# theo2021/OnDA

Hardware: AMD Instinct MI355X
Metric: adaptation-step images/sec (fwd+bwd+proto) 512x1024 bs=4 (higher is better)
Workload: dtype f32 (f16x2 split emulation); 1 GPU; hybrid_switch adaptation step (step + update_ema), 1024x512, bs=4 per micro-batch, 1 micro-batch(es) per GPU and optimizer step, dynamic branch, DeepLabV2-ResNet50 ProDA head, random-init weights; global_batch=4, parallelism=dp1, branch=dynamic, micro_batches_per_gpu=1, inputs=resident in HBM

## Files before the change

include/onda_hip.h:

```cpp
#ifndef ONDA_HIP_H
#define ONDA_HIP_H

#include <stdint.h>

#ifdef __cplusplus
extern "C" {
#endif

typedef void* onda_stream_t;

#define ONDA_OK 0
#define ONDA_EINVAL (-1)
#define ONDA_EALIGN (-2)

typedef struct OndaConv {
  int B, Hi, Wi, Cin;
  int Ho, Wo, Cout;
  int kh, kw, stride, dil, pad;
  int ldx;
  int ldy;
  int ldr;
  int out_os;
  int Hf, Wf;
  int relu;
// ... 83 lines not shown
int onda_conv2d_wgrad(const float* x, const float* dy, float* slabs, int lddy, int splitk,
                      const OndaConv* c, onda_stream_t s);
int onda_wgrad_reduce(const float* slabs, float* dw, int splitk, int Cout, int taps, int Cin,
                      int Cout_real, int Cin_real, int flat_k, int accumulate, onda_stream_t s);

int onda_pack_weight_fwd(const float* w_oihw, float* dst, int Cout, int Cin, int taps, int Cout_pad, int Kp,
                         onda_stream_t s);
int onda_pack_weight_dgrad(const float* w_oihw, float* dst, int Cout, int Cin, int taps, int Cout_pad,
                           onda_stream_t s);

int onda_stem_im2col(const float* x_nchw, float* col, int B, int H, int W, int Ho, int Wo, int Kp, onda_stream_t s);

int onda_bn_finalize(const float* partials, int tiles, int C, int64_t count, float eps, float* mean, float* invstd,
                     float* running_mean, float* running_var, int64_t* num_batches_tracked, float momentum,
                     onda_stream_t s);
int onda_bn_stats(const float* x, int64_t M, int C, int ldx, float* partials, int* tiles_out, onda_stream_t s);
int onda_bn_apply(const float* x, const float* mean, const float* invstd, const float* gamma, const float* beta,
                  const float* residual, float* out, int64_t M, int C, int relu, float* amax, onda_stream_t s);
int onda_bn_fold(const float* gamma, const float* beta, const float* running_mean, const float* running_var,
                 float eps, float* scale, float* shift, int C, onda_stream_t s);
int64_t onda_bn_bwd_ws(int64_t M, int C);
int onda_bn_bwd(const float* dout, const float* out, const float* x, const float* mean, const float* invstd,
                const float* gamma, float* dx, float* dres, float* ws, int64_t M, int C, int relu, float* amax, onda_stream_t s);

int64_t onda_gn_ws(int B, int64_t HW, int C);
int onda_gn_fwd(const float* x, int ldx, const float* gamma, const float* beta, const float* chmul, float* out, int ldo,
                float* mean, float* rstd, float* ws, int B, int64_t HW, int C, int groups, float eps, int relu,
                float* amax ,
                onda_stream_t s);
int onda_gn_bwd(const float* dout, int lddo, const float* out, int ldo, const float* x, int ldx, const float* gamma,
                const float* chmul, const float* mean, const float* rstd, float* dx, float* dgamma, float* dbeta,
                float* ws, int B, int64_t HW, int C, int groups, int relu, onda_stream_t s);

int onda_maxpool_fwd(const float* x, float* y, uint8_t* idx, int B, int Hi, int Wi, int C, int Ho, int Wo,
                     onda_stream_t s);
int onda_maxpool_fwd_limbs(const float* x, const float* xamax, void* yl, uint8_t* idx, int B, int Hi, int Wi, int C, int Ho, int Wo,
                           onda_stream_t s);
int onda_maxpool_bwd(const float* dy, const uint8_t* idx, float* dx, int B, int Hi, int Wi, int C, int Ho, int Wo,
                     onda_stream_t s);

int64_t onda_colsum_ws(int B, int64_t HW, int C);
int onda_colsum(const float* x, int ldx, const float* y, int ldy, float* out, float alpha, float* ws, int B,
                int64_t HW, int C, onda_stream_t s);
int onda_se_fc_fwd(const float* pooled, const float* w1, const float* b1, const float* w2, const float* b2,
                   float* hidden, float* gate, int B, int C, int R, onda_stream_t s);
int onda_se_fc_bwd(const float* dgate, const float* pooled, const float* hidden, const float* gate, const float* w1,
                   const float* w2, float* dw1, float* db1, float* dw2, float* db2, float* dpooled, float* ws,
                   float dpooled_scale, int B, int C, int R, onda_stream_t s);
int onda_chan_scale(const float* x, const float* gate, const float* add, float* out, int B, int64_t HW, int C,
                    onda_stream_t s);
int onda_chan_scale_limbs(const float* x, const float* gate, void* out, int64_t out_plane, const float* x_amax, int B, int64_t HW,
                          int C, onda_stream_t s);

int onda_upsample_fwd(const float* logits, int ldl, float* out_nchw, int B, int h, int w, int K, int H, int W,
                      onda_stream_t s);
int onda_upsample_bwd(const float* dout_nchw, float* dlogits, int ldl, int B, int h, int w, int K, int H, int W,
                      onda_stream_t s);
int onda_upsample_ce_fused(int w, int W);
int64_t onda_upsample_ce_ws(int B, int H, int W);
int onda_upsample_ce_fwd(const float* logits, int ldl, const uint8_t* labels, float* result, float* ws, int B, int h, int w, int K,
                         int H, int W, onda_stream_t s);
int64_t onda_upsample_ce_bwd_ws(int B, int w, int K, int H);
int onda_upsample_ce_bwd(const float* logits, int ldl, const uint8_t* labels, const float* result, const float* gscale, float w_ce,
                         float* dlogits, float* ws, int B, int h, int w, int K, int H, int W, onda_stream_t s);
int onda_upsample_argmax(const float* logits, int ldl, uint8_t* cls, int B, int h, int w, int K, int H, int W,
                         onda_stream_t s);
// ... 75 lines not shown
```

onda_amd/_lib.py:

```python
import ctypes
import os
from ctypes import POINTER, Structure, c_char_p, c_float, c_int, c_int64, c_void_p

HERE = os.path.dirname(os.path.abspath(__file__))
LIB_PATH = os.environ.get("ONDA_LIB_PATH") or os.path.join(HERE, "libonda_hip.so")

P = c_void_p
I, L, F = c_int, c_int64, c_float


class OndaConv(Structure):
    _fields_ = [(n, c_int) for n in ("B Hi Wi Cin Ho Wo Cout kh kw stride dil pad ldx ldy ldr out_os Hf Wf relu").split()] + \
               [("run_if", c_void_p), ("stat_split", c_int64), ("plain_schedule", c_int), ("pix_table", c_void_p),
                ("pix_stride", c_int64)]


class OndaSwitchCfg(Structure):
    _fields_ = [("limit", c_int), ("level_kind", c_int), ("use_exp", c_int), ("pad_", c_int), ("exp_const", ctypes.c_double),
                ("one_minus_exp_const", ctypes.c_double), ("taps_total", ctypes.c_double), ("gray_lo", ctypes.c_double),
                ("gray_hi", ctypes.c_double), ("dev_threshold", ctypes.c_double)]


class OndaLimbOut(Structure):
    _fields_ = [("out", c_void_p), ("out_plane", c_int64), ("out_bound", c_void_p), ("out_amax", c_void_p), ("kb", c_void_p),
# ... 32 lines not shown
    "onda_switch_step": (I, [P, P, P, I, P, POINTER(OndaSwitchCfg), P, P]),
    "onda_select_prior": (I, [P, P, F, P, F, P, L, P]),
    "onda_gate_scalar": (I, [P, P, P, P]),
    "onda_conv_l2_variant": (I, [L, I]),
    "onda_conv_l2_kernel_id": (I, [L, I, I, I]),
    "onda_conv_l2_tiles_m": (I, [L, I, I, I]),
    "onda_conv_l2_tiles_m_split": (I, [L, I, I, I, L, I, POINTER(c_int)]),
    "onda_conv_l2_live_fraction": (ctypes.c_double, [POINTER(OndaConv), I]),
    "onda_conv_wgrad_l2_live_fraction": (ctypes.c_double, [POINTER(OndaConv), I]),
    "onda_conv_wgrad_l2_variant": (I, [I, I]),
    "onda_conv2d_wgrad_l2_table_stride": (L, [POINTER(OndaConv)]),
    "onda_conv2d_wgrad_l2_table": (I, [POINTER(OndaConv), P, P]),
    "onda_conv2d_wgrad_l2": (I, [P, L, P, P, L, P, P, I, I, POINTER(OndaConv), P]),
    "onda_conv2d_fwd_l2": (I, [P, L, P, P, P, P, P, P, P, P, I, P, P, POINTER(OndaConv), P]),
    "onda_bn_finalize_l2": (I, [P, I, I, L, F, P, P, P, P, P, F, P, P, P, I, P, P, L, I, I, P, I, P]),
    "onda_bn_apply_l2": (I, [P, P, P, P, P, P, L, P, P, L, P, L, I, I, P, L, P]),
    "onda_bn_bwd_l2_ws": (L, [L, I]),
    "onda_bn_train_l2": (I, [P, P, I, F, P, P, P, P, P, F, P, P, P, P, I, P, P, P, L, I, P, L, I, I, P]),
    "onda_bn_bwd_l2": (I, [P, P, L, P, P, P, P, P, P, L, P, P, P, L, I, I, P, L, I, P]),
    "onda_conv2d_wgrad": (I, [P, P, P, I, I, POINTER(OndaConv), P]),
    "onda_wgrad_reduce": (I, [P, P, I, I, I, I, I, I, I, I, P]),
    "onda_pack_weight_fwd": (I, [P, P, I, I, I, I, I, P]),
    "onda_pack_weight_dgrad": (I, [P, P, I, I, I, I, P]),
    "onda_stem_im2col": (I, [P, P, I, I, I, I, I, I, P]),
    "onda_bn_finalize": (I, [P, I, I, L, F, P, P, P, P, P, F, P]),
    "onda_bn_stats": (I, [P, L, I, I, P, POINTER(c_int), P]),
    "onda_bn_apply": (I, [P, P, P, P, P, P, P, L, I, I, P, P]),
    "onda_bn_fold": (I, [P, P, P, P, F, P, P, I, P]),
    "onda_bn_bwd_ws": (L, [L, I]),
    "onda_bn_bwd": (I, [P, P, P, P, P, P, P, P, P, L, I, I, P, P]),
    "onda_gn_ws": (L, [I, L, I]),
    "onda_gn_fwd": (I, [P, I, P, P, P, P, I, P, P, P, I, L, I, I, F, I, P, P]),
    "onda_gn_bwd": (I, [P, I, P, I, P, I, P, P, P, P, P, P, P, P, I, L, I, I, I, P]),
    "onda_maxpool_fwd": (I, [P, P, P, I, I, I, I, I, I, P]),
    "onda_maxpool_fwd_limbs": (I, [P, P, P, P, I, I, I, I, I, I, P]),
    "onda_maxpool_bwd": (I, [P, P, P, I, I, I, I, I, I, P]),
    "onda_colsum_ws": (L, [I, L, I]),
    "onda_colsum": (I, [P, I, P, I, P, F, P, I, L, I, P]),
    "onda_se_fc_fwd": (I, [P, P, P, P, P, P, P, I, I, I, P]),
    "onda_se_fc_bwd": (I, [P, P, P, P, P, P, P, P, P, P, P, P, F, I, I, I, P]),
    "onda_chan_scale": (I, [P, P, P, P, I, L, I, P]),
    "onda_chan_scale_limbs": (I, [P, P, P, L, P, I, L, I, P]),
    "onda_upsample_fwd": (I, [P, I, P, I, I, I, I, I, I, P]),
    "onda_upsample_bwd": (I, [P, P, I, I, I, I, I, I, I, P]),
    "onda_upsample_argmax": (I, [P, I, P, I, I, I, I, I, I, P]),
    "onda_upsample_ce_fused": (I, [I, I]),
    "onda_upsample_ce_ws": (L, [I, I, I]),
    "onda_upsample_ce_fwd": (I, [P, I, P, P, P, I, I, I, I, I, I, P]),
    "onda_upsample_ce_bwd_ws": (L, [I, I, I, I]),
    "onda_upsample_ce_bwd": (I, [P, I, P, P, P, F, P, P, I, I, I, I, I, I, P]),
    "onda_upsample_argmax_hist": (I, [P, I, P, P, P, I, I, I, I, I, I, P]),
    "onda_softmax_stats": (I, [P, I, P, I, P, P, P, L, I, P]),
    "onda_seg_loss_fwd": (I, [P, I, P, P, P, L, I, P]),
    "onda_seg_loss_bwd": (I, [P, I, P, P, P, F, F, F, P, L, I, P]),
    "onda_target_loss_fwd": (I, [P, I, P, I, F, F, F, F, P, P, L, I, P]),
    "onda_target_loss_bwd": (I, [P, I, P, I, F, F, F, F, P, P, P, L, I, P]),
    "onda_proto_sigma": (I, [P, P, P, P, I, I, P]),
    "onda_proto_assign_blocks": (I, [L]),
    "onda_proto_assign": (I, [P, I, P, I, P, P, I, F, F, P, P, P, P, L, I, I, P]),
    "onda_proto_distances": (I, [P, I, P, P, I, P, L, I, I, P]),
    "onda_proto_sums_ws": (L, [L, I, I]),
    "onda_proto_class_sums": (I, [P, I, P, P, P, P, L, I, I, P]),
    "onda_proto_ema": (I, [P, P, P, P, F, I, I, P]),
    "onda_proto_append": (I, [P, P, P, P, P, I, I, P]),
    "onda_sgd_multi": (I, [P, I, F, F, F, L, P]),
    "onda_ema_multi": (I, [P, I, L, P]),
# ... 46 lines not shown
```

onda_amd/csrc/norm.hip:

```cpp
#include "common.h"

namespace {

struct ColPlan {
  int cx, ry, gridx, chunks;
  int64_t rows_per_chunk;
};

static inline ColPlan col_plan(int B, int64_t HW, int C) {
  ColPlan p;
  const int c4 = C / 4;
  p.cx = 1;
  while (p.cx < c4 && p.cx < 64) p.cx <<= 1;
  p.ry = 256 / p.cx;
  p.gridx = (c4 + p.cx - 1) / p.cx;
  int64_t target = 2048 / ((int64_t)B * p.gridx);
  if (target < 1) target = 1;
  int64_t rpc = (HW + target - 1) / target;
  const int64_t min_rows = (int64_t)p.ry * 8;
  if (rpc < min_rows) rpc = min_rows;
  p.rows_per_chunk = rpc;
  p.chunks = (int)((HW + rpc - 1) / rpc);
  return p;
}
// ... 241 lines not shown
  if (threadIdx.x != 0) return;
  s1 = ((red[0][0] + red[0][1]) + red[0][2]) + red[0][3];
  s2 = ((red[1][0] + red[1][1]) + red[1][2]) + red[1][3];
  const double mu = s1 / count;
  double var = s2 / count - mu * mu;
  if (var < 0.0) var = 0.0;
  mean[idx] = (float)mu;
  rstd[idx] = (float)(1.0 / sqrt(var + (double)eps));
}

__global__ __launch_bounds__(256) void gn_apply_kernel(const float* __restrict__ x, int ldx,
                                                       const float* __restrict__ gamma, const float* __restrict__ beta,
                                                       const float* __restrict__ chmul, float* __restrict__ out,
                                                       int ldo, const float* __restrict__ mean,
                                                       const float* __restrict__ rstd, int64_t HW, int C, int groups,
                                                       size_t total4, int relu, float* __restrict__ amax) {
  const int c4 = C / 4, cpg = C / groups;
  float mx = 0.f;
  for (size_t e = (size_t)blockIdx.x * blockDim.x + threadIdx.x; e < total4; e += (size_t)gridDim.x * blockDim.x) {
    const int col = (int)(e % c4) * 4;
    const size_t row = e / c4;
    const int b = (int)(row / HW);
    const int gi = b * groups + col / cpg;
    f32x4 v = (LD4(x + row * ldx + col) - mean[gi]) * rstd[gi] * LD4(gamma + col) + LD4(beta + col);
    if (relu) {
#pragma unroll
      for (int j = 0; j < 4; ++j) v[j] = fmaxf(v[j], 0.f);
    }
    if (chmul) v *= LD4(chmul + (size_t)b * C + col);
    *reinterpret_cast<f32x4*>(out + row * ldo + col) = v;
    mx = fmaxf(fmaxf(mx, fmaxf(fabsf(v[0]), fabsf(v[1]))), fmaxf(fabsf(v[2]), fabsf(v[3])));
  }
  if (amax != nullptr) amax_update(amax, mx);
}

__global__ __launch_bounds__(256) void pair_finalize_kernel(const float* __restrict__ partials, int chunks, int B,
                                                            int C, float* __restrict__ AB) {
  const int lane = threadIdx.x & 63;
  const int i = blockIdx.x * 4 + (threadIdx.x >> 6);
  if (i >= B * C) return;
  const int b = i / C, ch = i % C;
  double s1 = 0.0, s2 = 0.0;
  for (int k = lane; k < chunks; k += 64) {
    const size_t base = (((size_t)b * chunks + k) * 2) * C + ch;
    s1 += (double)partials[base];
    s2 += (double)partials[base + C];
  }
  s1 = wave_sum_d(s1);
  s2 = wave_sum_d(s2);
  if (lane == 0) {
    AB[((size_t)b * 2 + 0) * C + ch] = (float)s1;
    AB[((size_t)b * 2 + 1) * C + ch] = (float)s2;
  }
}

__global__ void gn_bwd_group_kernel(const float* __restrict__ AB, int B, int C, int groups,
                                    const float* __restrict__ gamma, float* __restrict__ dgamma,
                                    float* __restrict__ dbeta, float* __restrict__ gsum ) {
  for (int ch = threadIdx.x; ch < C; ch += blockDim.x) {
    float da = 0.f, db = 0.f;
    for (int b = 0; b < B; ++b) {
      db += AB[((size_t)b * 2 + 0) * C + ch];
      da += AB[((size_t)b * 2 + 1) * C + ch];
    }
    if (dgamma) dgamma[ch] = da;
    if (dbeta) dbeta[ch] = db;
// ... 12 lines not shown
  }
}

__global__ __launch_bounds__(256) void gn_bwd_apply_kernel(const float* __restrict__ dout, int lddo,
                                                           const float* __restrict__ out, int ldo,
                                                           const float* __restrict__ x, int ldx,
                                                           const float* __restrict__ gamma,
                                                           const float* __restrict__ chmul,
                                                           const float* __restrict__ mean,
                                                           const float* __restrict__ rstd,
                                                           const float* __restrict__ gsum, float* __restrict__ dx,
                                                           int64_t HW, int C, int groups, size_t total4, float inv_n,
                                                           int relu) {
  const int c4 = C / 4, cpg = C / groups;
  for (size_t e = (size_t)blockIdx.x * blockDim.x + threadIdx.x; e < total4; e += (size_t)gridDim.x * blockDim.x) {
    const int col = (int)(e % c4) * 4;
    const size_t row = e / c4;
    const int b = (int)(row / HW);
    const int gi = b * groups + col / cpg;
    f32x4 g = LD4(dout + row * lddo + col);
    if (relu) {
      const f32x4 ov = LD4(out + row * ldo + col);
#pragma unroll
      for (int j = 0; j < 4; ++j) g[j] = ov[j] > 0.f ? g[j] : 0.f;
    }
    if (chmul) g *= LD4(chmul + (size_t)b * C + col);
    const float rs = rstd[gi];
    const f32x4 xh = (LD4(x + row * ldx + col) - mean[gi]) * rs;
    const f32x4 v = rs * (LD4(gamma + col) * g - (gsum[gi * 2] + xh * gsum[gi * 2 + 1]) * inv_n);
    *reinterpret_cast<f32x4*>(dx + row * C + col) = v;
  }
}

__global__ __launch_bounds__(256) void colsum_finalize_kernel(const float* __restrict__ partials, int chunks, int B,
                                                              int C, float alpha, float* out) {
  const int lane = threadIdx.x & 63;
  const int i = blockIdx.x * 4 + (threadIdx.x >> 6);
  if (i >= B * C) return;
  const int b = i / C, ch = i % C;
  double s = 0.0;
  for (int k = lane; k < chunks; k += 64) s += (double)partials[(((size_t)b * chunks + k) * 2) * C + ch];
  s = wave_sum_d(s);
  if (lane == 0) out[i] = (float)(s * (double)alpha);
}

static inline unsigned ew_grid(size_t total4) {
  size_t g = (total4 + 255) / 256;
  if (g > 8192) g = 8192;
  if (g < 1) g = 1;
  return (unsigned)g;
}

}

extern "C" {

int onda_bn_finalize(const float* partials, int tiles, int C, int64_t count, float eps, float* mean, float* invstd,
                     float* running_mean, float* running_var, int64_t* nbt, float momentum, onda_stream_t s) {
  ONDA_REQUIRE(partials && mean && invstd && tiles >= 1 && C >= 1 && count >= 1);
  hipLaunchKernelGGL(bn_finalize_kernel, dim3((C + 3) / 4), dim3(256), 0, ONDA_STREAM(s), partials, tiles, C,
                     (double)count, eps, mean, invstd, running_mean, running_var, nbt, momentum);
  return ONDA_LAUNCH_RESULT();
}

int onda_bn_stats(const float* x, int64_t M, int C, int ldx, float* partials, int* tiles_out, onda_stream_t s) {
  ONDA_REQUIRE(x && partials && tiles_out && C % 4 == 0 && ldx % 4 == 0);
// ... 54 lines not shown
  const ColPlan p = col_plan(B, HW, C);
  SqStats f{x, HW, ldx};
  int rc = launch_colreduce(f, B, HW, C, ws, p, ONDA_STREAM(s));
  if (rc) return rc;
  hipLaunchKernelGGL(gn_finalize_kernel, dim3(B * groups), dim3(256), 0, ONDA_STREAM(s), ws, p.chunks, B,
                     C, groups, (double)HW * (C / groups), eps, mean, rstd);
  const size_t total4 = (size_t)B * HW * C / 4;
  hipLaunchKernelGGL(gn_apply_kernel, dim3(ew_grid(total4)), dim3(256), 0, ONDA_STREAM(s), x, ldx, gamma, beta, chmul,
                     out, ldo, mean, rstd, HW, C, groups, total4, relu, amax);
  return ONDA_LAUNCH_RESULT();
}

int onda_gn_bwd(const float* dout, int lddo, const float* out, int ldo, const float* x, int ldx, const float* gamma,
                const float* chmul, const float* mean, const float* rstd, float* dx, float* dgamma, float* dbeta,
                float* ws, int B, int64_t HW, int C, int groups, int relu, onda_stream_t s) {
  ONDA_REQUIRE(dout && x && gamma && mean && rstd && dx && ws && (!relu || out));
  ONDA_REQUIRE(C % groups == 0 && (C / groups) % 4 == 0 && ldx % 4 == 0 && lddo % 4 == 0);
  const ColPlan p = col_plan(B, HW, C);
  float* AB = ws + (size_t)B * p.chunks * 2 * C;
  float* gsum = AB + (size_t)B * 2 * C;
  GnBwdRed f{dout, out, x, chmul, mean, rstd, HW, lddo, ldo, ldx, C, groups, relu};
  int rc = launch_colreduce(f, B, HW, C, ws, p, ONDA_STREAM(s));
  if (rc) return rc;
  hipLaunchKernelGGL(pair_finalize_kernel, dim3((B * C + 3) / 4), dim3(256), 0, ONDA_STREAM(s), ws, p.chunks, B, C, AB);
  hipLaunchKernelGGL(gn_bwd_group_kernel, dim3(1), dim3(256), 0, ONDA_STREAM(s), AB, B, C, groups, gamma, dgamma, dbeta,
                     gsum);
  const size_t total4 = (size_t)B * HW * C / 4;
  hipLaunchKernelGGL(gn_bwd_apply_kernel, dim3(ew_grid(total4)), dim3(256), 0, ONDA_STREAM(s), dout, lddo, out, ldo, x,
                     ldx, gamma, chmul, mean, rstd, gsum, dx, HW, C, groups, total4,
                     (float)(1.0 / ((double)HW * (C / groups))), relu);
  return ONDA_LAUNCH_RESULT();
}

int64_t onda_colsum_ws(int B, int64_t HW, int C) {
  const ColPlan p = col_plan(B, HW, C);
  return (int64_t)B * p.chunks * 2 * C;
}

int onda_colsum(const float* x, int ldx, const float* y, int ldy, float* out, float alpha, float* ws, int B,
                int64_t HW, int C, onda_stream_t s) {
  ONDA_REQUIRE(x && out && ws && C % 4 == 0 && ldx % 4 == 0 && (!y || ldy % 4 == 0));
  const ColPlan p = col_plan(B, HW, C);
  ProdSum f{x, y, HW, ldx, ldy};
  int rc = launch_colreduce(f, B, HW, C, ws, p, ONDA_STREAM(s));
  if (rc) return rc;
  hipLaunchKernelGGL(colsum_finalize_kernel, dim3((B * C + 3) / 4), dim3(256), 0, ONDA_STREAM(s), ws, p.chunks, B, C,
                     alpha, out);
  return ONDA_LAUNCH_RESULT();
}

}
```

onda_amd/ops/conv.py:

```python
import ctypes
import os
from ctypes import byref

import torch

from .. import _lib
from .._lib import OndaConv, OndaLimbOut, call, query
from . import _state
from ._state import BN_EPS, GN_EPS, GN_GROUPS, HEAD_PAD, STEM_K
from .core import _conv_ws, _desc, _group_split, _l2_name, _launch, _p, _require_cuda, _stream, as_nhwc, conv_out_size, nhwc_ld
from .limbs import H2Weight, Limbs, amax_slot, is_limb_only, known_amax, limb_only, limbs_of, tag_amax
from .tables import _table


def _use_l2(wp, cin):
    return isinstance(wp, H2Weight) and _state.H2_PATH == "dma" and cin % 32 == 0


def _pack_h2(weight, rows_pad, kp, dgrad, cout_pad):
    cout, cin, kh, kw = weight.shape
    w = weight.detach().contiguous()
    slot = known_amax(weight)
    if slot is None:
        slot = amax_slot(weight.device, long_lived=True)
# ... 264 lines not shown
            "onda_conv2d_wgrad", _p(x), _p(dy), _p(slabs), nhwc_ld(dy), sk, byref(d), _stream(),
            tag=("wgrad", M, Co, Cin, k, stride, dil, sk))


def _wgrad_finish(slabs, into, sk, Co, taps, Cin, cout_real, cin_real, flat_k, k, device):
    if into is not None:
        call("onda_wgrad_reduce", _p(slabs), _p(into), sk, Co, taps, Cin, cout_real, cin_real, flat_k, 1, _stream())
        return None
    if flat_k:
        dw = torch.empty(cout_real, cin_real, 7, 7, device=device, dtype=torch.float32)
    else:
        dw = torch.empty(cout_real, cin_real, k, k, device=device, dtype=torch.float32)
    call("onda_wgrad_reduce", _p(slabs), _p(dw), sk, Co, taps, Cin, cout_real, cin_real, flat_k, 0, _stream())
    return dw


def _accumulate_target(weight):
    g = weight.grad
    if g is not None and g.is_contiguous() and g.dtype == torch.float32 and g.shape == weight.shape:
        return g
    return None


def colsum(x, y=None, alpha=1.0, per_image=False):
    B, H, W, C = x.shape
    nb, hw = (B, H * W) if per_image else (1, B * H * W)
    ws = torch.empty(query("onda_colsum_ws", nb, hw, C), device=x.device, dtype=torch.float32)
    out = torch.empty(nb, C, device=x.device, dtype=torch.float32)
    call("onda_colsum", _p(x), nhwc_ld(x), _p(y), nhwc_ld(y) if y is not None else 0, _p(out), float(alpha), _p(ws),
         nb, hw, C, _stream())
    return out if per_image else out[0]


class _PackCache:

    def __init__(self):
        self.key_f = self.key_d = None
        self.fwd = self.dgrad = None

    @staticmethod
    def _key(w):
        return (w.data_ptr(), w._version, w.device, _state.CONV_MODE)

    def get_fwd(self, w, cout_pad=None, kp=None):
        k = self._key(w)
        if self.key_f != k:
            self.fwd, self.key_f = pack_weight_fwd(w, cout_pad, kp), k
        return self.fwd

    def get_dgrad(self, w, cout_pad=None):
        k = self._key(w)
        if self.key_d != k:
            self.dgrad, self.key_d = pack_weight_dgrad(w, cout_pad), k
        return self.dgrad

    def __deepcopy__(self, memo):
        return _PackCache()


class ModelPacker:

    def __init__(self, convs):
        self.convs = [c for c in convs if c.weight.shape[0] % 32 == 0 and c.weight.shape[1] % 32 == 0]
        self.bufs = {}

    def refresh(self, need_dgrad):
# ... 33 lines not shown
            self._keep.append(w)
        table = _table(ents, _lib.OndaPackEntry, dev)
        call("onda_pack_weights_h2_multi", _p(table), len(ents), biggest, _stream())
        self._keep = []


class Conv2dFn(torch.autograd.Function):

    @staticmethod
    def forward(ctx, x, weight, bias, cache, stride, dil, pad, want_stats, cout_pad):
        cout, cin, k, _ = weight.shape
        co = cout_pad or cout
        wp = cache.get_fwd(weight, cout_pad)
        y, stats, _tiles = conv_forward(x, wp, k, stride, dil, pad, co, shift=_pad_vec(bias, co), want_stats=want_stats)
        ctx.save_for_backward(x, weight)
        ctx.xscale = known_amax(x)
        hit = getattr(x, "_onda_limbs", None)
        ctx.xlimbs = hit[1] if hit is not None and hit[0] == x._version else None
        ctx.weight_param = weight
        ctx.sink = _sink_of(x) if ctx.needs_input_grad[0] else None
        ctx.cache, ctx.geom, ctx.has_bias = cache, (k, stride, dil, pad, cout, cin, cout_pad), bias is not None
        ctx.set_materialize_grads(False)
        if want_stats:
            ctx.mark_non_differentiable(stats)
            return y, stats
        return y, None

    @staticmethod
    def backward(ctx, dy, _dstats):
        if dy is None:
            return (None,) * 9
        x, weight = ctx.saved_tensors
        k, stride, dil, pad, cout, cin, cout_pad = ctx.geom
        if not is_limb_only(dy):
            dy = as_nhwc(dy)
        dx = dw = db = None
        if ctx.needs_input_grad[0]:
            sink = ctx.sink
            wpd = ctx.cache.get_dgrad(weight, cout_pad)
            if sink is not None and sink.buf is not None:
                conv_dgrad(dy, wpd, k, stride, dil, pad, cin, x.shape[1:3], accumulate=sink.buf)
                _sink_done(sink)
            else:
                dx = _sink_give(sink, conv_dgrad(dy, wpd, k, stride, dil, pad, cin, x.shape[1:3]), True)
        if ctx.needs_input_grad[1]:
            into = _accumulate_target(ctx.weight_param)
            dw = conv_wgrad(x, dy, k, stride, dil, pad, cout, cin, into=into, xscale=ctx.xscale, xlimbs=ctx.xlimbs)
            if into is not None and _state.GRAD_READY is not None:
                _state.GRAD_READY(ctx.weight_param)
        if ctx.has_bias and ctx.needs_input_grad[2]:
            db = colsum(dy)[:cout]
        return dx, dw, db, None, None, None, None, None, None


def _pad_vec(v, n):
    if v is None or v.numel() == n:
        return v
    out = torch.zeros(n, device=v.device, dtype=v.dtype)
    out[: v.numel()] = v.detach()
    return out


def stem_patches(x_nchw, Ho, Wo, l2):
    hit = getattr(x_nchw, "_onda_patches", None)
    key = (x_nchw._version, bool(l2), Ho, Wo)
    if hit is not None and hit[0] == key:
        return hit[1]
    B, _, H, W = x_nchw.shape
    dev = x_nchw.device
    if l2:
        amax = amax_slot(dev)
        call("onda_absmax", _p(x_nchw), 1, x_nchw.numel(), x_nchw.numel(), _p(amax), _stream())
        M = B * Ho * Wo
        planes = torch.empty(2, M, STEM_K, device=dev, dtype=torch.float16)
        call("onda_stem_im2col_l2", _p(x_nchw), _p(amax), _p(planes), M * STEM_K, B, H, W, Ho, Wo, STEM_K, _stream())
        col = limb_only((B, Ho, Wo, STEM_K), dev, Limbs(planes, amax, STEM_K, M * STEM_K))
    else:
        col = torch.empty(B, Ho, Wo, STEM_K, device=dev, dtype=torch.float32)
        call("onda_stem_im2col", _p(x_nchw), _p(col), B, H, W, Ho, Wo, STEM_K, _stream())
    try:
        x_nchw._onda_patches = (key, col)
    except AttributeError:
        pass
    return col
# ... 53 lines not shown
```

onda_amd/ops/limbs.py:

```python
import ctypes
import os
from ctypes import byref

import torch

from .. import _lib
from .._lib import OndaConv, OndaLimbOut, call, query
from . import _state
from ._state import BN_EPS, GN_EPS, GN_GROUPS, HEAD_PAD, STEM_K
from .core import _p, _stream, nhwc_ld


class H2Weight:
    __slots__ = ("limbs", "amax")

    def __init__(self, limbs, amax):
        self.limbs, self.amax = limbs, amax


_AMAX_POOL = {}


AMAX_SLOTS = 2048
AMAX_POOL_TENSORS = 16384
# ... 12 lines not shown


def amax_slot(device, long_lived=False):
    key = (str(device), bool(long_lived))
    pool = _AMAX_POOL.get(key)
    if pool is None or pool[1] + AMAX_SLOTS > pool[0].numel():
        pool = _AMAX_POOL[key] = _new_amax_pool(device, WEIGHT_POOL_TENSORS if long_lived else AMAX_POOL_TENSORS)
    if pool[2] is not None:
        cur = torch.cuda.current_stream()
        if cur.cuda_stream not in pool[3]:
            cur.wait_event(pool[2])
            pool[3].add(cur.cuda_stream)
    i = pool[1]
    pool[1] = i + AMAX_SLOTS
    return pool[0][i:i + AMAX_SLOTS]


def reserve_amax_slots(device, n):
    pool = _AMAX_POOL.get((str(device), False))
    if pool is None or pool[1] + n * AMAX_SLOTS > pool[0].numel():
        _AMAX_POOL[(str(device), False)] = _new_amax_pool(device)


def tag_amax(t, slot):
    try:
        t._onda_scale = (t._version, slot)
    except AttributeError:
        pass
    return t


def known_amax(t):
    hit = getattr(t, "_onda_scale", None)
    return hit[1] if hit is not None and hit[0] == t._version else None


def activation_scale(x):
    slot = known_amax(x)
    if slot is not None:
        return slot
    B, H, W, C = x.shape
    slot = amax_slot(x.device)
    call("onda_absmax", _p(x), B * H * W, C, nhwc_ld(x), _p(slot), _stream())
    tag_amax(x, slot)
    return slot


class Limbs:
    __slots__ = ("planes", "amax", "ld", "plane", "true_amax")

    def __init__(self, planes, amax, ld, plane, true_amax=None):
        self.planes, self.amax, self.ld, self.plane = planes, amax, ld, plane
        self.true_amax = true_amax if true_amax is not None else amax


def activation_limbs(x):
    hit = getattr(x, "_onda_limbs", None)
    if hit is not None and hit[0] == x._version:
        return hit[1]
    amax = activation_scale(x)
    B, H, W, C = x.shape
    rows = B * H * W
    planes = torch.empty(2, rows, C, device=x.device, dtype=torch.float16)
    call("onda_split_h2", _p(x), rows, C, nhwc_ld(x), _p(planes), C, rows * C, _p(amax), _stream())
    lb = Limbs(planes, amax, C, rows * C)
    try:
# ... 52 lines not shown
```

onda_amd/ops/norm.py:

```python
import ctypes
import os
from ctypes import byref

import torch

from .. import _lib
from .._lib import OndaConv, OndaLimbOut, call, query
from . import _state
from ._state import BN_EPS, GN_EPS, GN_GROUPS, HEAD_PAD, STEM_K
from .core import _group_split, _p, _stream, as_nhwc, nhwc_ld
from .limbs import Limbs, _stat_tile_rows, amax_slot, is_limb_only, known_amax, limb_mode, limb_only, limbs_of, tag_amax
from .conv import _sink_give, _sink_of, colsum


class BNTrainFn(torch.autograd.Function):

    @staticmethod
    def _groups(B, H, W):
        split, M = _group_split(B, H, W), B * H * W
        return [(0, M)] if not split else [(0, split), (split, M - split)]

    @staticmethod
    def forward(ctx, y, stats, gamma, beta, residual, relu, running, momentum):
        B, H, W, C = y.shape
        groups = BNTrainFn._groups(B, H, W)
        G = len(groups)
        mean = torch.empty(G, C, device=y.device, dtype=torch.float32)
        invstd = torch.empty_like(mean)
        out = torch.empty_like(y)
        res = as_nhwc(residual) if residual is not None else None
        if res is not None and nhwc_ld(res) != C:
            res = res.contiguous()
        if G > 1 and (nhwc_ld(y) != C or not y.is_contiguous()):
            raise RuntimeError("onda_amd: row groups need a dense conv output")
        amax = amax_slot(y.device) if _state.CONV_MODE == "f16x2" else None
        for g, (r0, rows) in enumerate(groups):
            part, nrows = stats, stats.shape[0]
            if G > 1:
                bm = _stat_tile_rows(stats)
                if groups[1][0] % bm == 0 and stats.shape[1] == 2:
                    ts = groups[1][0] // bm
                    part = stats[:ts] if g == 0 else stats[ts:]
                    nrows = part.shape[0]
                else:
                    part = torch.empty(query("onda_bn_bwd_ws", rows, C), device=y.device, dtype=torch.float32)
# ... 144 lines not shown
        ctx.save_for_backward(idx)
        ctx.in_shape = (B, Hi, Wi, C)
        if limbs and slot is not None and limb_mode(C):
            planes = torch.empty(2, B * Ho * Wo, C, device=x.device, dtype=torch.float16)
            call("onda_maxpool_fwd_limbs", _p(x), _p(slot), _p(planes), _p(idx), B, Hi, Wi, C, Ho, Wo, _stream())
            return limb_only((B, Ho, Wo, C), x.device, Limbs(planes, slot, C, B * Ho * Wo * C))
        y = torch.empty(B, Ho, Wo, C, device=x.device, dtype=torch.float32)
        call("onda_maxpool_fwd", _p(x), _p(y), _p(idx), B, Hi, Wi, C, Ho, Wo, _stream())
        if slot is not None:
            tag_amax(y, slot)
        return y

    @staticmethod
    def backward(ctx, dy):
        (idx,) = ctx.saved_tensors
        B, Hi, Wi, C = ctx.in_shape
        dy = dy.contiguous()
        dx = torch.empty(B, Hi, Wi, C, device=dy.device, dtype=torch.float32)
        call("onda_maxpool_bwd", _p(dy), _p(idx), _p(dx), B, Hi, Wi, C, dy.shape[1], dy.shape[2], _stream())
        return dx, None


class GNConcatFn(torch.autograd.Function):

    @staticmethod
    def forward(ctx, relu, chmul, *args):
        n = len(args) // 3
        ys, gammas, betas = args[:n], args[n:2 * n], args[2 * n:]
        B, H, W, C = ys[0].shape
        HW = H * W
        cat = torch.empty(B, H, W, C * n, device=ys[0].device, dtype=torch.float32)
        ws = torch.empty(query("onda_gn_ws", B, HW, C), device=cat.device, dtype=torch.float32)
        amax = amax_slot(cat.device) if _state.CONV_MODE == "f16x2" else None
        means, rstds = [], []
        for i in range(n):
            mean = torch.empty(B * GN_GROUPS, device=cat.device, dtype=torch.float32)
            rstd = torch.empty_like(mean)
            sl = cat[..., i * C:(i + 1) * C]
            call("onda_gn_fwd", _p(ys[i]), nhwc_ld(ys[i]), _p(gammas[i]), _p(betas[i]), _p(chmul), _p(sl), C * n,
                 _p(mean), _p(rstd), _p(ws), B, HW, C, GN_GROUPS, GN_EPS, int(relu), _p(amax), _stream())
            means.append(mean)
            rstds.append(rstd)
        if amax is not None:
            tag_amax(cat, amax)
        ctx.save_for_backward(cat, chmul, *ys, *gammas, *means, *rstds)
        ctx.n, ctx.relu = n, relu
        return cat

    @staticmethod
    def backward(ctx, dcat):
        n = ctx.n
        saved = ctx.saved_tensors
        cat, chmul = saved[0], saved[1]
        ys, gammas = saved[2:2 + n], saved[2 + n:2 + 2 * n]
        means, rstds = saved[2 + 2 * n:2 + 3 * n], saved[2 + 3 * n:2 + 4 * n]
        B, H, W, C = ys[0].shape
        HW = H * W
        dcat = as_nhwc(dcat)
        ldd = nhwc_ld(dcat)
        ws = torch.empty(query("onda_gn_ws", B, HW, C), device=cat.device, dtype=torch.float32)
        dys, dgs, dbs = [], [], []
        for i in range(n):
            dx = torch.empty(B, H, W, C, device=cat.device, dtype=torch.float32)
            dg = torch.empty(C, device=cat.device, dtype=torch.float32)
            db = torch.empty_like(dg)
            call("onda_gn_bwd", dcat.data_ptr() + 4 * i * C, ldd, cat.data_ptr() + 4 * i * C, C * n, _p(ys[i]),
                 nhwc_ld(ys[i]), _p(gammas[i]), _p(chmul), _p(means[i]), _p(rstds[i]), _p(dx), _p(dg), _p(db), _p(ws),
                 B, HW, C, GN_GROUPS, int(ctx.relu), _stream())
            dys.append(dx)
            dgs.append(dg)
            dbs.append(db)
        return (None, None, *dys, *dgs, *dbs)




class SEScaleFn(torch.autograd.Function):

    @staticmethod
    def forward(ctx, x, w1, b1, w2, b2):
        B, H, W, C = x.shape
        R = w1.shape[0]
        pooled = colsum(x, alpha=1.0 / (H * W), per_image=True)
        hidden = torch.empty(B, R, device=x.device, dtype=torch.float32)
        gate = torch.empty(B, C, device=x.device, dtype=torch.float32)
        call("onda_se_fc_fwd", _p(pooled), _p(w1), _p(b1), _p(w2), _p(b2), _p(hidden), _p(gate), B, C, R, _stream())
        slot = known_amax(x)
        if slot is not None and limb_mode(C) and x.is_contiguous():
            planes = torch.empty(2, B * H * W, C, device=x.device, dtype=torch.float16)
            call("onda_chan_scale_limbs", _p(x), _p(gate), _p(planes), B * H * W * C, _p(slot), B, H * W, C, _stream())
            out = limb_only((B, H, W, C), x.device, Limbs(planes, slot, C, B * H * W * C))
        else:
            out = torch.empty_like(x)
            call("onda_chan_scale", _p(x), _p(gate), None, _p(out), B, H * W, C, _stream())
        ctx.save_for_backward(x, pooled, hidden, gate, w1, w2)
        return out

    @staticmethod
    def backward(ctx, dout):
        x, pooled, hidden, gate, w1, w2 = ctx.saved_tensors
        B, H, W, C = x.shape
        R = w1.shape[0]
        dout = dout.contiguous()
        dgate = colsum(dout, x, per_image=True)
        dw1, db1 = torch.empty_like(w1), torch.empty(R, device=x.device, dtype=torch.float32)
        dw2, db2 = torch.empty_like(w2), torch.empty(C, device=x.device, dtype=torch.float32)
        dpooled = torch.empty(B, C, device=x.device, dtype=torch.float32)
        ws = torch.empty(B * R, device=x.device, dtype=torch.float32)
        call("onda_se_fc_bwd", _p(dgate), _p(pooled), _p(hidden), _p(gate), _p(w1), _p(w2), _p(dw1), _p(db1), _p(dw2),
             _p(db2), _p(dpooled), _p(ws), 1.0 / (H * W), B, C, R, _stream())
        dx = torch.empty_like(x)
        call("onda_chan_scale", _p(dout), _p(gate), _p(dpooled), _p(dx), B, H * W, C, _stream())
        return dx, dw1, db1, dw2, db2
```

Baseline: 42.43 images/s.

## Fuse per-channel column sums and amax into GroupNorm apply kernels

The GroupNorm forward and backward apply kernels now also write per-chunk column partial sums, and in backward an amax. Those partials are tagged on the output tensors and reused later. The SE pooling reads them instead of re-reading the concatenated activation, and the conv bias gradient uses the column sums of the GN backward dx instead of launching a separate colsum pass. This removes extra full-tensor read passes over large activations, at the cost of block reductions and partial-buffer writes inside the apply kernels.

```diff
diff --git a/include/onda_hip.h b/include/onda_hip.h
--- a/include/onda_hip.h
+++ b/include/onda_hip.h
@@ -139,6 +139,16 @@
                 const float* chmul, const float* mean, const float* rstd, float* dx, float* dgamma, float* dbeta,
                 float* ws, int B, int64_t HW, int C, int groups, int relu, onda_stream_t s);
 
+int onda_gn_colsum_chunks(int B, int64_t HW, int C);
+int onda_gn_fwd_colsum(const float* x, int ldx, const float* gamma, const float* beta, const float* chmul, float* out, int ldo,
+                       float* mean, float* rstd, float* ws, int B, int64_t HW, int C, int groups, float eps, int relu,
+                       float* amax, float* colpart, int ldp, onda_stream_t s);
+int onda_gn_bwd_colsum(const float* dout, int lddo, const float* out, int ldo, const float* x, int ldx, const float* gamma,
+                       const float* chmul, const float* mean, const float* rstd, float* dx, float* dgamma, float* dbeta,
+                       float* ws, int B, int64_t HW, int C, int groups, int relu, float* amax, float* colpart, int ldp,
+                       onda_stream_t s);
+int onda_colpart_finalize(const float* colpart, int chunks, int ldp, int B, int C, float alpha, float* out, onda_stream_t s);
+
 int onda_maxpool_fwd(const float* x, float* y, uint8_t* idx, int B, int Hi, int Wi, int C, int Ho, int Wo,
                      onda_stream_t s);
 int onda_maxpool_fwd_limbs(const float* x, const float* xamax, void* yl, uint8_t* idx, int B, int Hi, int Wi, int C, int Ho, int Wo,
diff --git a/onda_amd/_lib.py b/onda_amd/_lib.py
--- a/onda_amd/_lib.py
+++ b/onda_amd/_lib.py
@@ -88,6 +88,10 @@
     "onda_gn_ws": (L, [I, L, I]),
     "onda_gn_fwd": (I, [P, I, P, P, P, P, I, P, P, P, I, L, I, I, F, I, P, P]),
     "onda_gn_bwd": (I, [P, I, P, I, P, I, P, P, P, P, P, P, P, P, I, L, I, I, I, P]),
+    "onda_gn_colsum_chunks": (I, [I, L, I]),
+    "onda_gn_fwd_colsum": (I, [P, I, P, P, P, P, I, P, P, P, I, L, I, I, F, I, P, P, I, P]),
+    "onda_gn_bwd_colsum": (I, [P, I, P, I, P, I, P, P, P, P, P, P, P, P, I, L, I, I, I, P, P, I, P]),
+    "onda_colpart_finalize": (I, [P, I, I, I, I, F, P, P]),
     "onda_maxpool_fwd": (I, [P, P, P, I, I, I, I, I, I, P]),
     "onda_maxpool_fwd_limbs": (I, [P, P, P, P, I, I, I, I, I, I, P]),
     "onda_maxpool_bwd": (I, [P, P, P, I, I, I, I, I, I, P]),
diff --git a/onda_amd/csrc/norm.hip b/onda_amd/csrc/norm.hip
--- a/onda_amd/csrc/norm.hip
+++ b/onda_amd/csrc/norm.hip
@@ -297,6 +297,72 @@
     mx = fmaxf(fmaxf(mx, fmaxf(fabsf(v[0]), fabsf(v[1]))), fmaxf(fabsf(v[2]), fabsf(v[3])));
   }
   if (amax != nullptr) amax_update(amax, mx);
+}
+
+__device__ __forceinline__ void amax_update_grid3(float* amax, float m, float* red) {
+  m = wave_max(m);
+  if ((threadIdx.x & 63) == 0) red[threadIdx.x >> 6] = m;
+  __syncthreads();
+  if (threadIdx.x == 0) {
+    m = fmaxf(fmaxf(red[0], red[1]), fmaxf(red[2], red[3]));
+    const unsigned wg = blockIdx.x + gridDim.x * (blockIdx.y + gridDim.y * blockIdx.z);
+    if (m > 0.f) atomicMax(reinterpret_cast<unsigned*>(amax) + (wg & (ONDA_AMAX_SLOTS - 1)) * AMAX_STRIDE, __float_as_uint(m));
+  }
+}
+
+__device__ __forceinline__ void colpart_store(f32x4 s, f32x4* red, int cx, int tx, int ty, int col, int C,
+                                              float* __restrict__ colpart, int ldp) {
+  const int ry_n = 256 / cx;
+  red[threadIdx.x] = s;
+  __syncthreads();
+  if (ty == 0 && col < C) {
+    for (int y = 1; y < ry_n; ++y) s += red[y * cx + tx];
+    *reinterpret_cast<f32x4*>(colpart + ((size_t)blockIdx.z * gridDim.y + blockIdx.y) * ldp + col) = s;
+  }
+}
+
+__global__ __launch_bounds__(256) void gn_apply_colsum_kernel(const float* __restrict__ x, int ldx,
+                                                              const float* __restrict__ gamma,
+                                                              const float* __restrict__ beta,
+                                                              const float* __restrict__ chmul, float* __restrict__ out,
+                                                              int ldo, const float* __restrict__ mean,
+                                                              const float* __restrict__ rstd, int64_t HW, int C, int groups,
+                                                              int cx, int64_t rows_per_chunk, int relu,
+                                                              float* __restrict__ amax, float* __restrict__ colpart,
+                                                              int ldp) {
+  __shared__ f32x4 red[256];
+  __shared__ float amax_red[4];
+  const int t = threadIdx.x;
+  const int ry_n = 256 / cx;
+  const int tx = t % cx, ty = t / cx;
+  const int col = (blockIdx.x * cx + tx) * 4;
+  const int b = blockIdx.z;
+  const int64_t r0 = (int64_t)blockIdx.y * rows_per_chunk;
+  const int64_t r1 = min(HW, r0 + rows_per_chunk);
+  f32x4 s = {0.f, 0.f, 0.f, 0.f};
+  float mx = 0.f;
+  if (col < C) {
+    const int gi = b * groups + col / (C / groups);
+    const float mu = mean[gi], rs = rstd[gi];
+    const f32x4 ga = LD4(gamma + col), be = LD4(beta + col);
+    f32x4 cm = {1.f, 1.f, 1.f, 1.f};
+    if (chmul) cm = LD4(chmul + (size_t)b * C + col);
+#pragma unroll 4
+    for (int64_t r = r0 + ty; r < r1; r += ry_n) {
+      const size_t row = (size_t)b * HW + r;
+      f32x4 v = (LD4(x + row * ldx + col) - mu) * rs * ga + be;
+      if (relu) {
+#pragma unroll
+        for (int j = 0; j < 4; ++j) v[j] = fmaxf(v[j], 0.f);
+      }
+      if (chmul) v *= cm;
+      *reinterpret_cast<f32x4*>(out + row * ldo + col) = v;
+      s += v;
+      mx = fmaxf(fmaxf(mx, fmaxf(fabsf(v[0]), fabsf(v[1]))), fmaxf(fabsf(v[2]), fabsf(v[3])));
+    }
+  }
+  colpart_store(s, red, cx, tx, ty, col, C, colpart, ldp);
+  if (amax != nullptr) amax_update_grid3(amax, mx, amax_red);
 }
 
 __global__ __launch_bounds__(256) void pair_finalize_kernel(const float* __restrict__ partials, int chunks, int B,
@@ -375,6 +441,61 @@
   }
 }
 
+__global__ __launch_bounds__(256) void gn_bwd_apply_colsum_kernel(
+    const float* __restrict__ dout, int lddo, const float* __restrict__ out, int ldo, const float* __restrict__ x, int ldx,
+    const float* __restrict__ gamma, const float* __restrict__ chmul, const float* __restrict__ mean,
+    const float* __restrict__ rstd, const float* __restrict__ gsum, float* __restrict__ dx, int64_t HW, int C, int groups,
+    int cx, int64_t rows_per_chunk, float inv_n, int relu, float* __restrict__ amax, float* __restrict__ colpart, int ldp) {
+  __shared__ f32x4 red[256];
+  __shared__ float amax_red[4];
+  const int t = threadIdx.x;
+  const int ry_n = 256 / cx;
+  const int tx = t % cx, ty = t / cx;
+  const int col = (blockIdx.x * cx + tx) * 4;
+  const int b = blockIdx.z;
+  const int64_t r0 = (int64_t)blockIdx.y * rows_per_chunk;
+  const int64_t r1 = min(HW, r0 + rows_per_chunk);
+  f32x4 s = {0.f, 0.f, 0.f, 0.f};
+  float mx = 0.f;
+  if (col < C) {
+    const int gi = b * groups + col / (C / groups);
+    const float mu = mean[gi], rs = rstd[gi], g0 = gsum[gi * 2], g1 = gsum[gi * 2 + 1];
+    const f32x4 ga = LD4(gamma + col);
+    f32x4 cm = {1.f, 1.f, 1.f, 1.f};
+    if (chmul) cm = LD4(chmul + (size_t)b * C + col);
+#pragma unroll 4
+    for (int64_t r = r0 + ty; r < r1; r += ry_n) {
+      const size_t row = (size_t)b * HW + r;
+      f32x4 g = LD4(dout + row * lddo + col);
+      if (relu) {
+        const f32x4 ov = LD4(out + row * ldo + col);
+#pragma unroll
+        for (int j = 0; j < 4; ++j) g[j] = ov[j] > 0.f ? g[j] : 0.f;
+      }
+      if (chmul) g *= cm;
+      const f32x4 xh = (LD4(x + row * ldx + col) - mu) * rs;
+      const f32x4 v = rs * (ga * g - (g0 + xh * g1) * inv_n);
+      *reinterpret_cast<f32x4*>(dx + row * C + col) = v;
+      s += v;
+      mx = fmaxf(fmaxf(mx, fmaxf(fabsf(v[0]), fabsf(v[1]))), fmaxf(fabsf(v[2]), fabsf(v[3])));
+    }
+  }
+  colpart_store(s, red, cx, tx, ty, col, C, colpart, ldp);
+  if (amax != nullptr) amax_update_grid3(amax, mx, amax_red);
+}
+
+__global__ __launch_bounds__(256) void colpart_finalize_kernel(const float* __restrict__ colpart, int chunks, int ldp,
+                                                               int B, int C, float alpha, float* __restrict__ out) {
+  const int lane = threadIdx.x & 63;
+  const int i = blockIdx.x * 4 + (threadIdx.x >> 6);
+  if (i >= B * C) return;
+  const int b = i / C, ch = i % C;
+  double s = 0.0;
+  for (int k = lane; k < chunks; k += 64) s += (double)colpart[((size_t)b * chunks + k) * ldp + ch];
+  s = wave_sum_d(s);
+  if (lane == 0) out[i] = (float)(s * (double)alpha);
+}
+
 __global__ __launch_bounds__(256) void colsum_finalize_kernel(const float* __restrict__ partials, int chunks, int B,
                                                               int C, float alpha, float* out) {
   const int lane = threadIdx.x & 63;
@@ -495,6 +616,54 @@
   return ONDA_LAUNCH_RESULT();
 }
 
+int onda_gn_colsum_chunks(int B, int64_t HW, int C) { return col_plan(B, HW, C).chunks; }
+
+int onda_gn_fwd_colsum(const float* x, int ldx, const float* gamma, const float* beta, const float* chmul, float* out, int ldo,
+                       float* mean, float* rstd, float* ws, int B, int64_t HW, int C, int groups, float eps, int relu,
+                       float* amax, float* colpart, int ldp, onda_stream_t s) {
+  ONDA_REQUIRE(x && gamma && beta && out && mean && rstd && ws && colpart);
+  ONDA_REQUIRE(C % groups == 0 && (C / groups) % 4 == 0 && ldx % 4 == 0 && ldo % 4 == 0 && ldp % 4 == 0 && ldp >= C);
+  ONDA_REQUIRE(ONDA_ALIGNED16(colpart) && ONDA_ALIGNED16(out) && ONDA_ALIGNED16(x));
+  const ColPlan p = col_plan(B, HW, C);
+  SqStats f{x, HW, ldx};
+  int rc = launch_colreduce(f, B, HW, C, ws, p, ONDA_STREAM(s));
+  if (rc) return rc;
+  hipLaunchKernelGGL(gn_finalize_kernel, dim3(B * groups), dim3(256), 0, ONDA_STREAM(s), ws, p.chunks, B,
+                     C, groups, (double)HW * (C / groups), eps, mean, rstd);
+  hipLaunchKernelGGL(gn_apply_colsum_kernel, dim3(p.gridx, p.chunks, B), dim3(256), 0, ONDA_STREAM(s), x, ldx, gamma, beta,
+                     chmul, out, ldo, mean, rstd, HW, C, groups, p.cx, p.rows_per_chunk, relu, amax, colpart, ldp);
+  return ONDA_LAUNCH_RESULT();
+}
+
+int onda_gn_bwd_colsum(const float* dout, int lddo, const float* out, int ldo, const float* x, int ldx, const float* gamma,
+                       const float* chmul, const float* mean, const float* rstd, float* dx, float* dgamma, float* dbeta,
+                       float* ws, int B, int64_t HW, int C, int groups, int relu, float* amax, float* colpart, int ldp,
+                       onda_stream_t s) {
+  ONDA_REQUIRE(dout && x && gamma && mean && rstd && dx && ws && colpart && (!relu || out));
+  ONDA_REQUIRE(C % groups == 0 && (C / groups) % 4 == 0 && ldx % 4 == 0 && lddo % 4 == 0 && ldp % 4 == 0 && ldp >= C);
+  ONDA_REQUIRE(ONDA_ALIGNED16(colpart) && ONDA_ALIGNED16(dx) && ONDA_ALIGNED16(dout));
+  const ColPlan p = col_plan(B, HW, C);
+  float* AB = ws + (size_t)B * p.chunks * 2 * C;
+  float* gsum = AB + (size_t)B * 2 * C;
+  GnBwdRed f{dout, out, x, chmul, mean, rstd, HW, lddo, ldo, ldx, C, groups, relu};
+  int rc = launch_colreduce(f, B, HW, C, ws, p, ONDA_STREAM(s));
+  if (rc) return rc;
+  hipLaunchKernelGGL(pair_finalize_kernel, dim3((B * C + 3) / 4), dim3(256), 0, ONDA_STREAM(s), ws, p.chunks, B, C, AB);
+  hipLaunchKernelGGL(gn_bwd_group_kernel, dim3(1), dim3(256), 0, ONDA_STREAM(s), AB, B, C, groups, gamma, dgamma, dbeta,
+                     gsum);
+  hipLaunchKernelGGL(gn_bwd_apply_colsum_kernel, dim3(p.gridx, p.chunks, B), dim3(256), 0, ONDA_STREAM(s), dout, lddo, out,
+                     ldo, x, ldx, gamma, chmul, mean, rstd, gsum, dx, HW, C, groups, p.cx, p.rows_per_chunk,
+                     (float)(1.0 / ((double)HW * (C / groups))), relu, amax, colpart, ldp);
+  return ONDA_LAUNCH_RESULT();
+}
+
+int onda_colpart_finalize(const float* colpart, int chunks, int ldp, int B, int C, float alpha, float* out, onda_stream_t s) {
+  ONDA_REQUIRE(colpart && out && chunks >= 1 && B >= 1 && C >= 1 && ldp >= C);
+  hipLaunchKernelGGL(colpart_finalize_kernel, dim3((B * C + 3) / 4), dim3(256), 0, ONDA_STREAM(s), colpart, chunks, ldp, B,
+                     C, alpha, out);
+  return ONDA_LAUNCH_RESULT();
+}
+
 int64_t onda_colsum_ws(int B, int64_t HW, int C) {
   const ColPlan p = col_plan(B, HW, C);
   return (int64_t)B * p.chunks * 2 * C;
diff --git a/onda_amd/ops/conv.py b/onda_amd/ops/conv.py
--- a/onda_amd/ops/conv.py
+++ b/onda_amd/ops/conv.py
@@ -320,6 +320,19 @@
     return out if per_image else out[0]
 
 
+def tag_colsum(t, sums):
+    try:
+        t._onda_colsum = (t._version, sums)
+    except AttributeError:
+        pass
+    return t
+
+
+def known_colsum(t):
+    hit = getattr(t, "_onda_colsum", None)
+    return hit[1] if hit is not None and hit[0] == t._version else None
+
+
 class _PackCache:
 
     def __init__(self):
@@ -419,6 +432,7 @@
             return (None,) * 9
         x, weight = ctx.saved_tensors
         k, stride, dil, pad, cout, cin, cout_pad = ctx.geom
+        dy_sums = known_colsum(dy)
         if not is_limb_only(dy):
             dy = as_nhwc(dy)
         dx = dw = db = None
@@ -436,7 +450,7 @@
             if into is not None and _state.GRAD_READY is not None:
                 _state.GRAD_READY(ctx.weight_param)
         if ctx.has_bias and ctx.needs_input_grad[2]:
-            db = colsum(dy)[:cout]
+            db = (dy_sums if dy_sums is not None and dy_sums.numel() == dy.shape[3] else colsum(dy))[:cout]
         return dx, dw, db, None, None, None, None, None, None
 
 
diff --git a/onda_amd/ops/limbs.py b/onda_amd/ops/limbs.py
--- a/onda_amd/ops/limbs.py
+++ b/onda_amd/ops/limbs.py
@@ -68,6 +68,19 @@
 
 def known_amax(t):
     hit = getattr(t, "_onda_scale", None)
+    return hit[1] if hit is not None and hit[0] == t._version else None
+
+
+def tag_colpart(t, colpart):
+    try:
+        t._onda_colpart = (t._version, colpart)
+    except AttributeError:
+        pass
+    return t
+
+
+def known_colpart(t):
+    hit = getattr(t, "_onda_colpart", None)
     return hit[1] if hit is not None and hit[0] == t._version else None
 
 
diff --git a/onda_amd/ops/norm.py b/onda_amd/ops/norm.py
--- a/onda_amd/ops/norm.py
+++ b/onda_amd/ops/norm.py
@@ -9,8 +9,8 @@
 from . import _state
 from ._state import BN_EPS, GN_EPS, GN_GROUPS, HEAD_PAD, STEM_K
 from .core import _group_split, _p, _stream, as_nhwc, nhwc_ld
-from .limbs import Limbs, _stat_tile_rows, amax_slot, is_limb_only, known_amax, limb_mode, limb_only, limbs_of, tag_amax
-from .conv import _sink_give, _sink_of, colsum
+from .limbs import Limbs, _stat_tile_rows, amax_slot, is_limb_only, known_amax, known_colpart, limb_mode, limb_only, limbs_of, tag_amax, tag_colpart
+from .conv import _sink_give, _sink_of, colsum, known_colsum, tag_colsum
 
 
 class BNTrainFn(torch.autograd.Function):
@@ -221,17 +221,26 @@
         cat = torch.empty(B, H, W, C * n, device=ys[0].device, dtype=torch.float32)
         ws = torch.empty(query("onda_gn_ws", B, HW, C), device=cat.device, dtype=torch.float32)
         amax = amax_slot(cat.device) if _state.CONV_MODE == "f16x2" else None
+        chunks = query("onda_gn_colsum_chunks", B, HW, C) if n > 1 else 0
+        colpart = torch.empty(B, chunks, C * n, device=cat.device, dtype=torch.float32) if chunks else None
         means, rstds = [], []
         for i in range(n):
             mean = torch.empty(B * GN_GROUPS, device=cat.device, dtype=torch.float32)
             rstd = torch.empty_like(mean)
             sl = cat[..., i * C:(i + 1) * C]
-            call("onda_gn_fwd", _p(ys[i]), nhwc_ld(ys[i]), _p(gammas[i]), _p(betas[i]), _p(chmul), _p(sl), C * n,
-                 _p(mean), _p(rstd), _p(ws), B, HW, C, GN_GROUPS, GN_EPS, int(relu), _p(amax), _stream())
+            if colpart is not None:
+                call("onda_gn_fwd_colsum", _p(ys[i]), nhwc_ld(ys[i]), _p(gammas[i]), _p(betas[i]), _p(chmul), _p(sl), C * n,
+                     _p(mean), _p(rstd), _p(ws), B, HW, C, GN_GROUPS, GN_EPS, int(relu), _p(amax),
+                     colpart.data_ptr() + 4 * i * C, C * n, _stream())
+            else:
+                call("onda_gn_fwd", _p(ys[i]), nhwc_ld(ys[i]), _p(gammas[i]), _p(betas[i]), _p(chmul), _p(sl), C * n,
+                     _p(mean), _p(rstd), _p(ws), B, HW, C, GN_GROUPS, GN_EPS, int(relu), _p(amax), _stream())
             means.append(mean)
             rstds.append(rstd)
         if amax is not None:
             tag_amax(cat, amax)
+        if colpart is not None:
+            tag_colpart(cat, colpart)
         ctx.save_for_backward(cat, chmul, *ys, *gammas, *means, *rstds)
         ctx.n, ctx.relu = n, relu
         return cat
@@ -248,17 +257,26 @@
         dcat = as_nhwc(dcat)
         ldd = nhwc_ld(dcat)
         ws = torch.empty(query("onda_gn_ws", B, HW, C), device=cat.device, dtype=torch.float32)
+        chunks = query("onda_gn_colsum_chunks", B, HW, C)
+        colpart = torch.empty(B * chunks, C * n, device=cat.device, dtype=torch.float32)
         dys, dgs, dbs = [], [], []
         for i in range(n):
             dx = torch.empty(B, H, W, C, device=cat.device, dtype=torch.float32)
             dg = torch.empty(C, device=cat.device, dtype=torch.float32)
             db = torch.empty_like(dg)
-            call("onda_gn_bwd", dcat.data_ptr() + 4 * i * C, ldd, cat.data_ptr() + 4 * i * C, C * n, _p(ys[i]),
+            amax = amax_slot(cat.device) if _state.CONV_MODE == "f16x2" else None
+            call("onda_gn_bwd_colsum", dcat.data_ptr() + 4 * i * C, ldd, cat.data_ptr() + 4 * i * C, C * n, _p(ys[i]),
                  nhwc_ld(ys[i]), _p(gammas[i]), _p(chmul), _p(means[i]), _p(rstds[i]), _p(dx), _p(dg), _p(db), _p(ws),
-                 B, HW, C, GN_GROUPS, int(ctx.relu), _stream())
+                 B, HW, C, GN_GROUPS, int(ctx.relu), _p(amax), colpart.data_ptr() + 4 * i * C, C * n, _stream())
+            if amax is not None:
+                tag_amax(dx, amax)
             dys.append(dx)
             dgs.append(dg)
             dbs.append(db)
+        sums = torch.empty(C * n, device=cat.device, dtype=torch.float32)
+        call("onda_colpart_finalize", _p(colpart), B * chunks, C * n, 1, C * n, 1.0, _p(sums), _stream())
+        for i, dx in enumerate(dys):
+            tag_colsum(dx, sums[i * C:(i + 1) * C])
         return (None, None, *dys, *dgs, *dbs)
 
 
@@ -270,7 +288,12 @@
     def forward(ctx, x, w1, b1, w2, b2):
         B, H, W, C = x.shape
         R = w1.shape[0]
-        pooled = colsum(x, alpha=1.0 / (H * W), per_image=True)
+        colpart = known_colpart(x)
+        if colpart is not None and tuple(colpart.shape) == (B, colpart.shape[1], C):
+            pooled = torch.empty(B, C, device=x.device, dtype=torch.float32)
+            call("onda_colpart_finalize", _p(colpart), colpart.shape[1], C, B, C, 1.0 / (H * W), _p(pooled), _stream())
+        else:
+            pooled = colsum(x, alpha=1.0 / (H * W), per_image=True)
         hidden = torch.empty(B, R, device=x.device, dtype=torch.float32)
         gate = torch.empty(B, C, device=x.device, dtype=torch.float32)
         call("onda_se_fc_fwd", _p(pooled), _p(w1), _p(b1), _p(w2), _p(b2), _p(hidden), _p(gate), B, C, R, _stream())
```

New measurement: 42.59 images/s, median of 6. No clear change (+0.4%).
